# JeongsooP/RGB-no-more

Measured on AMD Instinct MI355X. Metric: images/sec JPEG-Ti DCT 512x512 train step, higher is better.
Workload: dtype bf16

## Files before the change

rgb-no-more_amd/csrc/vit_chain_bwd.hip:

```cpp
#include "common.h"
#include <string.h>
#include <type_traits>
#include "internal.h"
#include "ln_bwd_rows.h"
#include "chain_common.h"
#include "../../include/rgbnm.h"

namespace {

constexpr int E = 192, HID = 768, HD = 64, HEADS = 3, NTOK = 196, NTILE = 7, NPAD = 224, INNER = HEADS * HD, LDQ = 3 * INNER;
constexpr int NCW = 7, NTHREADS = 64 * (NCW + 1), CTHREADS = 64 * NCW, BM = 32 * NCW;
constexpr int ARR = NPAD * ROWB, SLOT = 24576, STAGE = 2 * SLOT, CH = 64, NCHUNK = HID / CH;
constexpr int CP = E + 4;
constexpr int SMEM = 163840;
constexpr int PIPE_P = 6, PIPE_M1 = 5, PIPE_X = 7;
constexpr int M_STG = 2 * STAGE;
constexpr int TILE = 32 * ROWB;
typedef rgbnm::LnBwdRows<CTHREADS, BM> LnBwd;
constexpr int RED_OFF = (BM * CP * 2 + 1023) / 1024 * 1024;
static_assert(RED_OFF + LnBwd::RED_BYTES <= 132096, "LDS");
constexpr int P_SLOT0 = 132096, P_SLOT1 = 0, P_TILES = 98304;
static_assert(P_SLOT0 + SLOT <= SMEM && P_TILES + NCW * TILE <= P_SLOT0, "LDS");
constexpr int A_Q = 0, A_K = ARR, A_V = 2 * ARR, A_G = 3 * ARR, A_L2 = 4 * ARR, A_D = A_L2 + NPAD * 4, A_STG = A_D + NPAD * 4;
constexpr int A_SIDE = A_STG + NCW * STG_WAVE;
static_assert(A_SIDE + NCW * 1024 <= SMEM, "LDS");
constexpr int X_SLOT0 = A_K, X_SLOT1 = A_K + SLOT, X_SLOT2 = 0, X_TILES = A_K + 2 * SLOT, X_TSET = NCW * TILE;
static_assert(X_SLOT1 + SLOT <= X_TILES && X_TILES + 3 * X_TSET <= SMEM && SLOT <= A_K, "LDS");

struct BwdBlk {
  const bf16* wimg;
  const float *ln1_g, *ln2_g;
  const bf16* x_in; const float *mean1, *rstd1;
  const bf16* qkv; const float* lse; const bf16* attn; const bf16* x_mid; const float *mean2, *rstd2; const bf16* gp;
  const bf16* dy;
  bf16* du; bf16* dx_mid; bf16* dqkv; bf16* dx;
  float *part2, *part1;
};
static_assert(sizeof(BwdBlk) == sizeof(rgbnm_chain_bwd_block), "rgbnm_chain_bwd_block layout");
constexpr int MAX_DEPTH = 12;
struct BwdArgs {
  BwdBlk blk[MAX_DEPTH]; bf16* dattn;
  int depth, nimg;
  float scale;
};

__device__ __forceinline__ void store_du(bf16* ptr, const bf16x8& v) { __builtin_nontemporal_store(v, reinterpret_cast<bf16x8*>(ptr)); }

__device__ __forceinline__ void dma_row_tiles(const bf16* __restrict__ src, int ld, unsigned char* dst, int lane) {
#pragma unroll 4
  for (int i = 0; i < 28; ++i) {
    const int row = 8 * i + (lane >> 3), pc = lane & 7;
    const int lc = pc ^ (row & 7);
    const int srow = row < NTOK ? row : NTOK - 1;
    __builtin_amdgcn_global_load_lds((glb_ptr)(src + (size_t)srow * ld + lc * 8), (lds_ptr)(dst + i * 1024), 16, 0, 0);
  }
}

__device__ __forceinline__ void tile_out(unsigned char* smem, unsigned stg, const u32x4& p0, const u32x4& p1, const u32x4& p2,
                                         const u32x4& p3, bf16* dst, int ld, int live) {
  const int ln = lane_id_here();
  const unsigned wo = stg + (unsigned)((ln & 31) * ROWB + (((ln >> 5) ^ (ln & 7)) << 4));
  *reinterpret_cast<u32x4*>(smem + wo) = p0;
  *reinterpret_cast<u32x4*>(smem + (wo ^ 32u)) = p1;
  *reinterpret_cast<u32x4*>(smem + (wo ^ 64u)) = p2;
  *reinterpret_cast<u32x4*>(smem + (wo ^ 96u)) = p3;
  own_tile_fence();
  const int rl = ln >> 3, seg = ln & 7;
  const unsigned ro = stg + (unsigned)(rl * ROWB + ((seg ^ rl) << 4));
  bf16* gp = dst + (size_t)rl * ld + seg * 8;
  u32x4 v[4];
#pragma unroll
  for (int i = 0; i < 4; ++i) v[i] = *reinterpret_cast<const u32x4*>(smem + ro + i * 8 * ROWB);
  if (live == 32) {
#pragma unroll
    for (int i = 0; i < 4; ++i) *reinterpret_cast<u32x4*>(gp + (size_t)i * 8 * ld) = v[i];
  } else {
#pragma unroll
    for (int i = 0; i < 4; ++i)
      if (i * 8 + rl < live) *reinterpret_cast<u32x4*>(gp + (size_t)i * 8 * ld) = v[i];
  }
  own_tile_fence();
}

__device__ __forceinline__ void tiles_write(const u32x4 (&v)[NTILE][4], bf16* __restrict__ g0, size_t ld, int lane) {
  const int rl = lane >> 3, seg = lane & 7;
#pragma unroll
  for (int wv = 0; wv < NTILE; ++wv)
#pragma unroll
    for (int i = 0; i < 4; ++i) {
      const int row = wv * 32 + i * 8 + rl;
      if (row < NTOK) *reinterpret_cast<u32x4*>(g0 + (size_t)row * ld + seg * 8) = v[wv][i];
    }
}

#ifdef CHAINB_PROF
__device__ unsigned long long g_chainb_prof[8 * 8 * 128];
#define CP_(i)                                                                                          \
  do {                                                                                                  \
    if (ib == CHAINB_PROF_BLK && blockIdx.x < 8) {                                                      \
      const unsigned long long t_ = __builtin_amdgcn_s_memtime();                                       \
      if ((threadIdx.x & 63) == 0) g_chainb_prof[(blockIdx.x * 8 + (threadIdx.x >> 6)) * 128 + (i)] = t_; \
    }                                                                                                   \
  } while (0)
#ifndef CHAINB_PROF_BLK
#define CHAINB_PROF_BLK 6
#endif
#else
#define CP_(i) do {} while (0)
#endif
#define BAR(s) do { CP_(2 * (s)); wg_barrier(); CP_(2 * (s) + 1); } while (0)
constexpr int B_M0 = 0;
constexpr int B_E2 = 12;
constexpr int B_P = 19;
constexpr int B_A = 24;
constexpr int B_X = 37;
constexpr int B_E1 = 46;
constexpr int B_END = 53;

__device__ __forceinline__ void ln_bwd_request(LnBwd& lnb, const bf16* X, const float* mean, const float* rstd, const bf16* R, int img,
                                               int w) {
  const int tid = w * 64 + lane_id_here();
  lnb.request_x(X, E, mean, rstd, img * NTOK, NTOK, tid);
  lnb.request_res(R, E, img * NTOK, NTOK, tid);
}
template <int B0>
__device__ __forceinline__ void ln_bwd_epilogue(unsigned char* smem, const f32x16 (&acc)[6], const bf16* X, const float* mean,
                                                const float* rstd, const bf16* R, const float* gamma, bf16* DX,
                                                float* part, int img, int w, int ib) {
  const int lane_ = lane_id_here();
  const int tid = w * 64 + lane_, rloc = w * 32 + (lane_ & 31), g = lane_ >> 5;
  LnBwd lnb;
  lnb.request_x(X, E, mean, rstd, img * NTOK, NTOK, tid);
  lnb.request_res(R, E, img * NTOK, NTOK, tid);
  wait_lds();
  BAR(B0);
  bf16* Cs = reinterpret_cast<bf16*>(smem);
#pragma unroll
  for (int b = 0; b < 6; ++b)
#pragma unroll
    for (int q = 0; q < 4; ++q) {
      const int nl = 32 * b + 8 * q + 4 * g;
      const f32x4 v = {acc[b][4 * q + 0], acc[b][4 * q + 1], acc[b][4 * q + 2], acc[b][4 * q + 3]};
      store4<bf16>(Cs + rloc * CP + nl, v);
    }
  wait_lds();
  BAR(B0 + 1);
  lnb.run<true>(Cs, CP, DX, E, gamma, true, part, img, reinterpret_cast<float*>(smem + RED_OFF), img * NTOK, NTOK, tid, Cs,
          [&](int k) { if (k == 0) BAR(B0 + 2); else if (k == 1) BAR(B0 + 3); else if (k == 2) BAR(B0 + 4); else BAR(B0 + 5); });
  wait_lds();
  BAR(B0 + 6);
}
__device__ __forceinline__ void read_own_rows(const unsigned char* smem, int w, Rows& x) {
  const int lane_ = lane_id_here();
  const unsigned char* rp = smem + (w * 32 + (lane_ & 31)) * (CP * 2) + 16 * (lane_ >> 5);
#pragma unroll
  for (int c = 0; c < 12; ++c) {
    const u32x2 lo = *reinterpret_cast<const u32x2*>(rp + 32 * c), hi = *reinterpret_cast<const u32x2*>(rp + 32 * c + 8);
    x.v[c] = u32x4{lo[0], lo[1], hi[0], hi[1]};
  }
}

__global__ __launch_bounds__(NTHREADS) void vit_chain_bwd_kernel(BwdArgs p) {
  extern __shared__ __attribute__((aligned(16))) unsigned char smem[];
  const int img = blockIdx.x;
  if (img >= p.nimg) return;
  const int w = __builtin_amdgcn_readfirstlane(threadIdx.x >> 6);
  const int depth = p.depth;

  if (w == NCW) {
    const int lane = threadIdx.x & 63;
    for (int ib = depth - 1; ib >= 0; --ib) {
      const BwdBlk& b = p.blk[ib];
      const unsigned char* wimg = reinterpret_cast<const unsigned char*>(b.wimg);
      dma_linear<48>(wimg, smem, lane);
      for (int c = 0; c < NCHUNK; ++c) {
        wait_vm<0>();
        BAR(B_M0 + c);
        if (c + 1 < NCHUNK) dma_linear<48>(wimg + (size_t)(c + 1) * STAGE, smem + ((c + 1) & 1) * STAGE, lane);
      }
      BAR(B_E2);
      dma_linear<24>(wimg + (size_t)NCHUNK * STAGE, smem + P_SLOT0, lane);
#pragma unroll
      for (int k = 1; k < 7; ++k) BAR(B_E2 + k);
      const bf16* qkv0 = b.qkv + (size_t)img * NTOK * LDQ;
      const bf16* do0 = p.dattn + (size_t)img * NTOK * INNER;
      bf16* dq0 = b.dqkv + (size_t)img * NTOK * LDQ;
      const unsigned char* stg0 = smem + A_STG;
      auto issue_kv = [&](int h) {
        dma_matrix_all(qkv0 + INNER + h * HD, LDQ, NTOK, smem + A_K, lane);
        dma_matrix_all(qkv0 + 2 * INNER + h * HD, LDQ, NTOK, smem + A_V, lane);
      };
      auto issue_q = [&](int h) { dma_matrix_all(qkv0 + h * HD, LDQ, NTOK, smem + A_Q, lane); };
      auto issue_g = [&](int h) { dma_matrix_all(do0 + h * HD, INNER, NTOK, smem + A_G, lane); };
      const unsigned char* xw = wimg + (size_t)NCHUNK * STAGE + 3 * SLOT;
      auto issue_xt = [&](int j) { dma_row_tiles(dq0 + j * 64, LDQ, smem + X_TILES + (j % 3) * X_TSET, lane); };
      wait_vm<0>();
      BAR(B_P);
      BAR(B_P + 1);
      dma_linear<24>(wimg + (size_t)NCHUNK * STAGE + SLOT, smem + P_SLOT1, lane);
      issue_kv(0);
      wait_vm<56>(); BAR(B_P + 2);
      dma_linear<24>(wimg + (size_t)NCHUNK * STAGE + 2 * SLOT, smem + P_SLOT0, lane);
      wait_vm<0>(); BAR(B_P + 3);
      issue_q(0);
      BAR(B_P + 4);
      {
        issue_g(0);
        wait_vm<0>();
        BAR(B_A);
        for (int h = 0; h < HEADS; ++h) {
          bf16* g0 = dq0 + h * HD;
          wait_vm<0>();
          BAR(B_A + 1 + 4 * h);
          u32x4 tq[NTILE][4];
          tiles_read<true>(stg0, NTOK, lane, tq);
          wait_lds();
          BAR(B_A + 2 + 4 * h);
          tiles_write(tq, g0, LDQ, lane);
          if (h + 1 < HEADS) issue_kv(h + 1);
          else {
            dma_linear<24>(xw, smem + X_SLOT0, lane);
            dma_linear<24>(xw + SLOT, smem + X_SLOT1, lane);
          }
          wait_vm<0>();
          BAR(B_A + 3 + 4 * h);
          tiles_read<true>(stg0, NTOK, lane, tq);
          wait_lds();
          BAR(B_A + 4 + 4 * h);
          tiles_write(tq, g0 + INNER, LDQ, lane);
          tiles_read<false>(smem + A_G, NTOK, lane, tq);
          wait_lds();
          if (h + 1 < HEADS) {
            issue_q(h + 1);
            issue_g(h + 1);
          } else {
            issue_xt(0);
          }
          tiles_write(tq, g0 + 2 * INNER, LDQ, lane);
        }
      }
      for (int j = 0; j < 9; ++j) {
        if (j == 0) wait_vm<28>();
        else if (j + 1 < 9) wait_vm<52>();
        else wait_vm<0>();
        BAR(B_X + j);
        if (j == 0) {
          issue_xt(1);
          dma_linear<24>(xw + 2 * SLOT, smem + X_SLOT2, lane);
          issue_xt(2);
        }
        if (j + 2 < 9 && j >= 1) {
          dma_linear<24>(xw + (size_t)(j + 2) * SLOT, smem + ((j + 2) % 3 == 0 ? X_SLOT0 : ((j + 2) % 3 == 1 ? X_SLOT1 : X_SLOT2)), lane);
          issue_xt(j + 2);
        }
      }
#pragma unroll
      for (int k = 0; k < 7; ++k) BAR(B_E1 + k);
      BAR(B_END);
    }
    return;
  }

  const int row0 = 32 * w;
  const int live = NTOK - row0 < 32 ? NTOK - row0 : 32;
  const size_t grow0 = (size_t)img * NTOK + row0;
  const float LOG2E = 1.4426950408889634f;
  const float c2 = p.scale * LOG2E;

  Rows dyf;
  {
    const int lane_ = lane_id_here();
    const int rloc = row0 + (lane_ & 31), tok = rloc < NTOK ? rloc : NTOK - 1;
    const bf16* yrow = p.blk[depth - 1].dy + ((size_t)img * NTOK + tok) * E + 8 * (lane_ >> 5);
#pragma unroll
    for (int c = 0; c < 12; ++c) dyf.v[c] = *reinterpret_cast<const u32x4*>(yrow + 16 * c);
  }

  for (int ib = depth - 1; ib >= 0; --ib) {
    const BwdBlk& b = p.blk[ib];
    f32x16 acc2[6];
#pragma unroll
    for (int bt = 0; bt < 6; ++bt)
#pragma unroll
      for (int r = 0; r < 16; ++r) acc2[bt][r] = 0.f;
    {
      const Geo L = fresh_geo();
      const int fl = L.fl;
      const int woff0 = L.l31 * (E * 2) + ((L.g ^ fl) << 4);
      const unsigned stg = (unsigned)(M_STG + w * 2 * TILE);
      bf16x8 gpraw[4];
      auto load_gp = [&](int chunk) {
        const int ln = lane_id_here();
#pragma unroll
        for (int i = 0; i < 4; ++i) {
          const int idx = ln + 64 * i, row = idx >> 3, vec = idx & 7;
          int rr = row0 + row;
          rr = rr < NTOK ? rr : NTOK - 1;
          const bf16x8* gsrc = reinterpret_cast<const bf16x8*>(b.gp + ((size_t)img * NTOK + rr) * HID + chunk * CH + vec * 8);
          gpraw[i] = *gsrc;
        }
      };
      load_gp(0);
      for (int chunk = 0; chunk < NCHUNK; ++chunk) {
        {
          const int ln = lane_id_here();
#pragma unroll
          for (int i = 0; i < 4; ++i) {
            const int idx = ln + 64 * i, row = idx >> 3, vec = idx & 7;
            *reinterpret_cast<bf16x8*>(smem + stg + row * ROWB + ((vec ^ (row & 7)) << 4)) = gpraw[i];
          }
        }
        if (chunk + 1 < NCHUNK) load_gp(chunk + 1);
        wait_lds();
        BAR(B_M0 + chunk);
        const unsigned st_off = (unsigned)((chunk & 1) * STAGE);
        const unsigned char* sW1 = smem + st_off;
        const unsigned w2o = opaque(st_off + (unsigned)(SLOT + L.l31 * ROWB + ((L.g ^ fl) << 4)));
        const unsigned two = opaque(stg + (unsigned)(L.l31 * ROWB + ((L.g ^ (L.l31 & 7)) << 4)));
#pragma unroll
        for (int ht = 0; ht < 2; ++ht) {
          f32x16 a1;
#pragma unroll
          for (int r = 0; r < 16; ++r) a1[r] = 0.f;
          int wbase = woff0 + ht * 32 * (E * 2);
          asm volatile("" : "+v"(wbase));
          {
            Frag<bf16> fb[12];
#pragma unroll
            for (int c = 0; c < 12; ++c)
              fb[c].v = *reinterpret_cast<const bf16x8*>(sW1 + ((wbase ^ ((c % 4) << 5)) + 128 * (c / 4)));
#pragma unroll
            for (int c = 0; c < 12; ++c) {
              Frag<bf16> fx;
              fx.v = as_bf16x8(dyf.v[c]);
              mma(a1, fb[c], fx);
            }
            __builtin_amdgcn_sched_group_barrier(0x100, PIPE_M1, 0);
#pragma unroll
            for (int i = 0; i < 12 - PIPE_M1; ++i) {
              __builtin_amdgcn_sched_group_barrier(0x008, 1, 0);
              __builtin_amdgcn_sched_group_barrier(0x100, 1, 0);
            }
#pragma unroll
            for (int i = 0; i < PIPE_M1; ++i) __builtin_amdgcn_sched_group_barrier(0x008, 1, 0);
            __builtin_amdgcn_sched_barrier(0);
          }
          Frag<bf16> fw2[12];
#pragma unroll
          for (int bt = 0; bt < 6; ++bt)
            fw2[bt].v = *reinterpret_cast<const bf16x8*>(smem + (w2o ^ (unsigned)((2 * ht) << 5)) + bt * 32 * ROWB);
          __builtin_amdgcn_sched_barrier(0);
          Frag<bf16> pg[2];
#pragma unroll
          for (int hs = 0; hs < 2; ++hs) {
            const unsigned to = two ^ (unsigned)((2 * ht + hs) << 5);
            const bf16x8 gpv = *reinterpret_cast<const bf16x8*>(smem + to);
            bf16x8 dv;
#pragma unroll
            for (int j = 0; j < 8; ++j) dv[j] = (bf16)((float)(bf16)a1[8 * hs + j] * (float)gpv[j]);
            pg[hs].v = dv;
            *reinterpret_cast<bf16x8*>(smem + to + TILE) = dv;
          }
          __builtin_amdgcn_sched_barrier(0);
#pragma unroll
          for (int bt = 0; bt < 6; ++bt)
            fw2[6 + bt].v = *reinterpret_cast<const bf16x8*>(smem + (w2o ^ (unsigned)((2 * ht + 1) << 5)) + bt * 32 * ROWB);
#pragma unroll
          for (int bt = 0; bt < 6; ++bt) mma(acc2[bt], fw2[bt], pg[0]);
#pragma unroll
          for (int bt = 0; bt < 6; ++bt) mma(acc2[bt], fw2[6 + bt], pg[1]);
#pragma unroll
          for (int i = 0; i < 6; ++i) {
            __builtin_amdgcn_sched_group_barrier(0x008, 1, 0);
            __builtin_amdgcn_sched_group_barrier(0x100, 1, 0);
          }
          __builtin_amdgcn_sched_group_barrier(0x008, 6, 0);
          __builtin_amdgcn_sched_barrier(0);
        }
        own_tile_fence();
        const int ln = lane_id_here();
        bf16x8 dv0[4];
#pragma unroll
        for (int i = 0; i < 4; ++i) {
          const int idx = ln + 64 * i, row = idx >> 3, vec = idx & 7;
          dv0[i] = *reinterpret_cast<const bf16x8*>(smem + stg + TILE + row * ROWB + ((vec ^ (row & 7)) << 4));
        }
        if (live == 32) {
#pragma unroll
          for (int i = 0; i < 4; ++i) {
            const int idx = ln + 64 * i, row = idx >> 3, vec = idx & 7;
            store_du(b.du + (grow0 + row) * HID + chunk * CH + vec * 8, dv0[i]);
          }
        } else {
#pragma unroll
          for (int i = 0; i < 4; ++i) {
            const int idx = ln + 64 * i, row = idx >> 3, vec = idx & 7;
            if (row < live) store_du(b.du + (grow0 + row) * HID + chunk * CH + vec * 8, dv0[i]);
          }
        }
      }
    }
    ln_bwd_epilogue<B_E2>(smem, acc2, b.x_mid, b.mean2, b.rstd2, b.dy, b.ln2_g, b.dx_mid, b.part2, img, w, ib);
    {
      const Geo L = fresh_geo();
      Rows dxf;
      read_own_rows(smem, w, dxf);
      wait_lds();
      BAR(B_P);
      const unsigned stg = (unsigned)(P_TILES + w * TILE);
#pragma unroll
      for (int h = 0; h < HEADS; ++h) {
        BAR(B_P + 1 + h);
        const unsigned char* sW = smem + (h == 1 ? P_SLOT1 : P_SLOT0);
        f32x16 acc[2];
#pragma unroll
        for (int ht = 0; ht < 2; ++ht)
#pragma unroll
          for (int r = 0; r < 16; ++r) acc[ht][r] = 0.f;
        gemm_k192x2<PIPE_P, true>(acc[0], acc[1], sW, dxf, L);
        u32x4 pc[4];
#pragma unroll
        for (int ht = 0; ht < 2; ++ht)
#pragma unroll
          for (int hs = 0; hs < 2; ++hs)
#pragma unroll
            for (int d = 0; d < 4; ++d) pc[2 * ht + hs][d] = pack2(acc[ht][8 * hs + 2 * d], acc[ht][8 * hs + 2 * d + 1]);
        tile_out(smem, stg, pc[0], pc[1], pc[2], pc[3], p.dattn + grow0 * INNER + h * HD, INNER, live);
      }
      asm volatile("s_waitcnt vmcnt(0)" ::: "memory");
      BAR(B_P + 4);
    }
    {
      unsigned char* Qs = smem + A_Q;
      unsigned char* Ks = smem + A_K;
      unsigned char* Vs = smem + A_V;
      unsigned char* Gs = smem + A_G;
      float* L2_s = reinterpret_cast<float*>(smem + A_L2);
      float* D_s = reinterpret_cast<float*>(smem + A_D);
      unsigned char* stg = smem + A_STG + w * STG_WAVE;
      const Geo L = fresh_geo();
      const int fl = L.fl;
      const unsigned rb0 = (unsigned)(L.l31 * ROWB + ((L.g ^ fl) << 4));
      const int row = row0 + L.l31;
      u32x4 qraw[4], graw[4], oraw[4];
      float lq = 0.f;
      const bf16* qkv0 = b.qkv + (size_t)img * NTOK * LDQ;
      const bf16* do0 = p.dattn + (size_t)img * NTOK * INNER;
      const bf16* o0 = b.attn + (size_t)img * NTOK * INNER;
      auto load_own_g = [&](int h) {
        const int lane_ = lane_id_here();
        const int seg = lane_ & 7;
#pragma unroll
        for (int i = 0; i < 4; ++i) {
          int r = row0 + i * 8 + (lane_ >> 3);
          r = r < NTOK ? r : NTOK - 1;
          graw[i] = *reinterpret_cast<const u32x4*>(do0 + (size_t)r * INNER + h * HD + seg * 8);
        }
      };
      unsigned char* qside = smem + A_SIDE + w * 1024;
      auto load_own_q = [&](int h) {
        const int lane_ = lane_id_here();
        const int seg = lane_ & 7;
#pragma unroll
        for (int i = 0; i < 4; ++i) {
          int r = row0 + i * 8 + (lane_ >> 3);
          r = r < NTOK ? r : NTOK - 1;
          const bf16* src = qkv0 + (size_t)r * LDQ + h * HD + seg * 8;
          if (i == 0) __builtin_amdgcn_global_load_lds((glb_ptr)src, (lds_ptr)qside, 16, 0, 0);
          else qraw[i] = *reinterpret_cast<const u32x4*>(src);
        }
      };
      auto load_own_o = [&](int h) {
        const int lane_ = lane_id_here();
        const int seg = lane_ & 7;
#pragma unroll
        for (int i = 0; i < 4; ++i) {
          int r = row0 + i * 8 + (lane_ >> 3);
          r = r < NTOK ? r : NTOK - 1;
          oraw[i] = *reinterpret_cast<const u32x4*>(o0 + (size_t)r * INNER + h * HD + seg * 8);
        }
        int rq_ = row0 + (lane_ & 31);
        rq_ = rq_ < NTOK ? rq_ : NTOK - 1;
        lq = b.lse[((size_t)img * HEADS + h) * NTOK + rq_];
      };
      load_own_g(0);
      load_own_q(0);
      load_own_o(0);
      BAR(B_A);
      for (int h = 0; h < HEADS; ++h) {
        const bool more = h + 1 < HEADS;
        asm volatile("s_waitcnt vmcnt(0)" ::: "memory");
        Frag<bf16> kf[4], vf[4];
        {
          f32x16 dq[2];
          Frag<bf16> qf[4], gf[4];
          const int rl = L.lane >> 3, seg = L.lane & 7;
#pragma unroll
          for (int i = 0; i < 4; ++i) {
            const bf16x8 gv = __builtin_bit_cast(bf16x8, graw[i]), ov = __builtin_bit_cast(bf16x8, oraw[i]);
            float d = 0.f;
#pragma unroll
            for (int e = 0; e < 8; ++e) d += (float)gv[e] * (float)ov[e];
            d += lane_xor1(d);
            d += lane_xor2(d);
            d += lane_xor4(d);
            if (seg == 0) D_s[row0 + i * 8 + rl] = d;
          }
          qraw[0] = *reinterpret_cast<const u32x4*>(qside + lane_id_here() * 16);
#pragma unroll
          for (int i = 0; i < 4; ++i) *reinterpret_cast<u32x4*>(stg + (i * 8 + rl) * STG_PITCH + seg * 16) = qraw[i];
          own_tile_fence();
#pragma unroll
          for (int c = 0; c < 4; ++c) qf[c].v = *reinterpret_cast<const bf16x8*>(stg + L.l31 * STG_PITCH + (2 * c + L.g) * 16);
          own_tile_fence();
#pragma unroll
          for (int i = 0; i < 4; ++i) *reinterpret_cast<u32x4*>(stg + (i * 8 + rl) * STG_PITCH + seg * 16) = graw[i];
          own_tile_fence();
#pragma unroll
          for (int c = 0; c < 4; ++c) gf[c].v = *reinterpret_cast<const bf16x8*>(stg + L.l31 * STG_PITCH + (2 * c + L.g) * 16);
          const float Dq = D_s[row];
          own_tile_fence();
          const float lq2 = lq * LOG2E;
          if (L.g == 0) L2_s[row] = lq2;
#pragma unroll
          for (int dt = 0; dt < 2; ++dt)
#pragma unroll
            for (int r = 0; r < 16; ++r) dq[dt][r] = 0.f;
          unsigned rb = rb0, tr = L.tr0;
          asm volatile("" : "+v"(rb), "+v"(tr));
          const unsigned kt = (unsigned)A_K + tr;
          TileLoop<NTILE>::run([&](auto tc) {
            constexpr int t = decltype(tc)::value;
            f32x16 sa, da;
#pragma unroll
            for (int r = 0; r < 16; ++r) { sa[r] = 0.f; da[r] = 0.f; }
            row_pair_mma(sa, da, Ks, Vs, rb, t, qf, gf);
            float ds[16];
#pragma unroll
            for (int r = 0; r < 16; ++r) {
              const float pr = __builtin_amdgcn_exp2f(fmaf(sa[r], c2, -lq2));
              ds[r] = pr * (da[r] - Dq);
            }
            if (t * 32 + 32 > NTOK) {
#pragma unroll
              for (int r = 0; r < 16; ++r)
                if (t * 32 + acc_row(r, L.lane) >= NTOK) ds[r] = 0.f;
            }
            Frag<bf16> kk[4];
            tfrag4<t>(kt, kk);
            Frag<bf16> sf = pfrag<bf16>(ds, 0);
            mma(dq[0], kk[0], sf);
            mma(dq[1], kk[1], sf);
            sf = pfrag<bf16>(ds, 1);
            mma(dq[0], kk[2], sf);
            mma(dq[1], kk[3], sf);
          });
          tile_park_private(stg, dq, p.scale, L);
#pragma unroll
          for (int c = 0; c < 4; ++c) {
            kf[c] = rowfrag_x(Ks, rb, w, c);
            vf[c] = rowfrag_x(Vs, rb, w, c);
          }
        }
        wait_lds();
        BAR(B_A + 1 + 4 * h);
        BAR(B_A + 2 + 4 * h);
        {
          f32x16 dk[2], dv[2];
#pragma unroll
          for (int dt = 0; dt < 2; ++dt)
#pragma unroll
            for (int r = 0; r < 16; ++r) { dk[dt][r] = 0.f; dv[dt][r] = 0.f; }
          unsigned rb = rb0, tr = L.tr0;
          asm volatile("" : "+v"(rb), "+v"(tr));
          const unsigned qt_ = (unsigned)A_Q + tr, gt_ = (unsigned)A_G + tr;
          TileLoop<NTILE>::run([&](auto tc) {
            constexpr int t = decltype(tc)::value;
            f32x16 sa, da;
#pragma unroll
            for (int r = 0; r < 16; ++r) { sa[r] = 0.f; da[r] = 0.f; }
            row_pair_mma(sa, da, Qs, Gs, rb, t, kf, vf);
            float pp[16], ds[16];
#pragma unroll
            for (int q4 = 0; q4 < 4; ++q4) {
              const f32x4 l4 = *reinterpret_cast<const f32x4*>(L2_s + t * 32 + 8 * q4 + 4 * L.g);
              const f32x4 d4 = *reinterpret_cast<const f32x4*>(D_s + t * 32 + 8 * q4 + 4 * L.g);
#pragma unroll
              for (int e = 0; e < 4; ++e) {
                const int r = 4 * q4 + e;
                const float pr = __builtin_amdgcn_exp2f(fmaf(sa[r], c2, -l4[e]));
                pp[r] = pr;
                ds[r] = pr * (da[r] - d4[e]);
              }
            }
            if (t * 32 + 32 > NTOK) {
#pragma unroll
              for (int r = 0; r < 16; ++r)
                if (t * 32 + acc_row(r, L.lane) >= NTOK) { pp[r] = 0.f; ds[r] = 0.f; }
            }
            Frag<bf16> gg[4];
            tfrag4<t>(gt_, gg);
            Frag<bf16> f = pfrag<bf16>(pp, 0);
            mma(dv[0], gg[0], f);
            mma(dv[1], gg[1], f);
            f = pfrag<bf16>(pp, 1);
            mma(dv[0], gg[2], f);
            mma(dv[1], gg[3], f);
            tfrag4<t>(qt_, gg);
            f = pfrag<bf16>(ds, 0);
            mma(dk[0], gg[0], f);
            mma(dk[1], gg[1], f);
            f = pfrag<bf16>(ds, 1);
            mma(dk[0], gg[2], f);
            mma(dk[1], gg[3], f);
          });
          if (more) load_own_g(h + 1);
          tile_park_private(stg, dk, p.scale, L);
          if (more) load_own_q(h + 1);
          wait_lds();
          BAR(B_A + 3 + 4 * h);
          tile_park_rows(Gs, w, dv, 1.0f);
        }
        if (more) load_own_o(h + 1);
        wait_lds();
        BAR(B_A + 4 + 4 * h);
      }
    }
    f32x16 accx[6];
#pragma unroll
    for (int bt = 0; bt < 6; ++bt)
#pragma unroll
      for (int r = 0; r < 16; ++r) accx[bt][r] = 0.f;
    for (int j = 0; j < 9; ++j) {
      BAR(B_X + j);
      const Geo L = fresh_geo();
      const int fl = L.fl;
      const int set = j % 3;
      const unsigned wo = opaque((unsigned)((set == 0 ? X_SLOT0 : (set == 1 ? X_SLOT1 : X_SLOT2)) + L.l31 * ROWB + ((L.g ^ fl) << 4)));
      const unsigned to = opaque((unsigned)(X_TILES + set * X_TSET + w * TILE + L.l31 * ROWB + ((L.g ^ (L.l31 & 7)) << 4)));
#pragma unroll
      for (int s = 0; s < 4; ++s) {
        Frag<bf16> fx, fw[6];
        fx.v = *reinterpret_cast<const bf16x8*>(smem + (to ^ (unsigned)(s << 5)));
#pragma unroll
        for (int bt = 0; bt < 6; ++bt)
          fw[bt].v = *reinterpret_cast<const bf16x8*>(smem + (wo ^ (unsigned)(s << 5)) + bt * 32 * ROWB);
#pragma unroll
        for (int bt = 0; bt < 6; ++bt) mma(accx[bt], fw[bt], fx);
      }
      __builtin_amdgcn_sched_group_barrier(0x100, PIPE_X, 0);
#pragma unroll
      for (int i = 0; i < 24; ++i) {
        __builtin_amdgcn_sched_group_barrier(0x008, 1, 0);
        if (i < 28 - PIPE_X) __builtin_amdgcn_sched_group_barrier(0x100, 1, 0);
      }
      __builtin_amdgcn_sched_barrier(0);
    }
    ln_bwd_epilogue<B_E1>(smem, accx, b.x_in, b.mean1, b.rstd1, b.dx_mid, b.ln1_g, b.dx, b.part1, img, w, ib);
    read_own_rows(smem, w, dyf);
    wait_lds();
    BAR(B_END);
  }
}

}

#ifdef CHAINB_PROF
extern "C" int rgbnm_chainb_prof_read(unsigned long long* host_out) {
  return hipMemcpyFromSymbol(host_out, HIP_SYMBOL(g_chainb_prof), sizeof(unsigned long long) * 8 * 8 * 128) == hipSuccess ? 0 : -1;
}
#endif

extern "C" {

size_t rgbnm_chain_bwd_block_bytes(void) { return sizeof(BwdBlk); }

int rgbnm_vit_chain_bwd(const rgbnm_vit_cfg* c, const rgbnm_chain_bwd_block* blocks, int depth, void* dattn, void* stream) {
  if (!c || !blocks || !dattn || depth <= 0) return RGBNM_EINVAL;
  if (c->dtype != RGBNM_DT_BF16 || c->E != E || c->heads != HEADS || c->N != NTOK || c->B < 1 || depth > MAX_DEPTH) return 1;
  BwdArgs p;
  memcpy(p.blk, blocks, sizeof(BwdBlk) * depth);
  p.dattn = (bf16*)dattn; p.depth = depth; p.nimg = c->B; p.scale = c->attn_scale;
  static DevOnce attr;
  if (attr.need()) {
    if (hipFuncSetAttribute((const void*)vit_chain_bwd_kernel, hipFuncAttributeMaxDynamicSharedMemorySize, SMEM) != hipSuccess)
      return RGBNM_ELAUNCH;
    attr.done();
  }
  const double tok = (double)c->B * NTOK;
  const double flops = depth * tok * 2.0 * (2.0 * E * HID + INNER * E + 3.0 * INNER * E + 4.0 * NTOK * INNER);
  const double bytes = depth * (tok * ((2.0 * HID + 5.0 * E + 2.0 * 3.0 * INNER) * 2.0 + 4 * 4 + HEADS * 4) + 36.0 * SLOT) + tok * E * 2.0;
  const int slot = rgbnm_trace_begin(TR_CHAIN_BWD, flops, bytes, (hipStream_t)stream);
  hipLaunchKernelGGL(vit_chain_bwd_kernel, dim3(c->B), dim3(NTHREADS), SMEM, (hipStream_t)stream, p);
  rgbnm_trace_end(slot, (hipStream_t)stream);
  LAUNCH_CHECK();
  return RGBNM_OK;
}

}
```

Baseline: 68000.

## Reorder projection heads so last-head dattn stays in LDS and registers

The backward projection now processes heads in a rotated order (1,2,0), so head 0's dattn tile is produced last. That tile is written straight into the attention G buffer in LDS and kept in registers (graw). This replaces the later global reload of dattn for head 0 and the DMA issue_g(0). It also drops a vmcnt(0) wait in favour of an LDS wait, and clamps row reads. Risks include correctness on padded rows, changed swizzle assumptions, and higher register pressure.

```diff
diff --git a/rgb-no-more_amd/csrc/vit_chain_bwd.hip b/rgb-no-more_amd/csrc/vit_chain_bwd.hip
--- a/rgb-no-more_amd/csrc/vit_chain_bwd.hip
+++ b/rgb-no-more_amd/csrc/vit_chain_bwd.hip
@@ -27,6 +27,8 @@
 constexpr int X_SLOT0 = A_K, X_SLOT1 = A_K + SLOT, X_SLOT2 = 0, X_TILES = A_K + 2 * SLOT, X_TSET = NCW * TILE;
 static_assert(X_SLOT1 + SLOT <= X_TILES && X_TILES + 3 * X_TSET <= SMEM && SLOT <= A_K, "LDS");
 
+constexpr int p_head(int s) { return (s + 1) % HEADS; }
+
 struct BwdBlk {
   const bf16* wimg;
   const float *ln1_g, *ln2_g;
@@ -71,6 +73,31 @@
   u32x4 v[4];
 #pragma unroll
   for (int i = 0; i < 4; ++i) v[i] = *reinterpret_cast<const u32x4*>(smem + ro + i * 8 * ROWB);
+  if (live == 32) {
+#pragma unroll
+    for (int i = 0; i < 4; ++i) *reinterpret_cast<u32x4*>(gp + (size_t)i * 8 * ld) = v[i];
+  } else {
+#pragma unroll
+    for (int i = 0; i < 4; ++i)
+      if (i * 8 + rl < live) *reinterpret_cast<u32x4*>(gp + (size_t)i * 8 * ld) = v[i];
+  }
+  own_tile_fence();
+}
+
+__device__ __forceinline__ void tile_keep_out(unsigned char* smem, unsigned rows, const u32x4& p0, const u32x4& p1, const u32x4& p2,
+                                              const u32x4& p3, u32x4 (&v)[4], bf16* dst, int ld, int live) {
+  const int ln = lane_id_here();
+  const unsigned wo = rows + (unsigned)((ln & 31) * ROWB + (((ln >> 5) ^ fswz(ln & 31)) << 4));
+  *reinterpret_cast<u32x4*>(smem + wo) = p0;
+  *reinterpret_cast<u32x4*>(smem + (wo ^ 32u)) = p1;
+  *reinterpret_cast<u32x4*>(smem + (wo ^ 64u)) = p2;
+  *reinterpret_cast<u32x4*>(smem + (wo ^ 96u)) = p3;
+  own_tile_fence();
+  const int rl = ln >> 3, seg = ln & 7;
+  bf16* gp = dst + (size_t)rl * ld + seg * 8;
+#pragma unroll
+  for (int i = 0; i < 4; ++i)
+    v[i] = *reinterpret_cast<const u32x4*>(smem + rows + (unsigned)((i * 8 + rl) * ROWB + ((seg ^ fswz(i * 8 + rl)) << 4)));
   if (live == 32) {
 #pragma unroll
     for (int i = 0; i < 4; ++i) *reinterpret_cast<u32x4*>(gp + (size_t)i * 8 * ld) = v[i];
@@ -150,9 +177,12 @@
   wait_lds();
   BAR(B0 + 6);
 }
+template <bool CLAMP = false>
 __device__ __forceinline__ void read_own_rows(const unsigned char* smem, int w, Rows& x) {
   const int lane_ = lane_id_here();
-  const unsigned char* rp = smem + (w * 32 + (lane_ & 31)) * (CP * 2) + 16 * (lane_ >> 5);
+  int r = w * 32 + (lane_ & 31);
+  if (CLAMP) r = r < NTOK ? r : NTOK - 1;
+  const unsigned char* rp = smem + r * (CP * 2) + 16 * (lane_ >> 5);
 #pragma unroll
   for (int c = 0; c < 12; ++c) {
     const u32x2 lo = *reinterpret_cast<const u32x2*>(rp + 32 * c), hi = *reinterpret_cast<const u32x2*>(rp + 32 * c + 8);
@@ -179,7 +209,7 @@
         if (c + 1 < NCHUNK) dma_linear<48>(wimg + (size_t)(c + 1) * STAGE, smem + ((c + 1) & 1) * STAGE, lane);
       }
       BAR(B_E2);
-      dma_linear<24>(wimg + (size_t)NCHUNK * STAGE, smem + P_SLOT0, lane);
+      dma_linear<24>(wimg + (size_t)NCHUNK * STAGE + p_head(0) * SLOT, smem + P_SLOT0, lane);
 #pragma unroll
       for (int k = 1; k < 7; ++k) BAR(B_E2 + k);
       const bf16* qkv0 = b.qkv + (size_t)img * NTOK * LDQ;
@@ -197,15 +227,14 @@
       wait_vm<0>();
       BAR(B_P);
       BAR(B_P + 1);
-      dma_linear<24>(wimg + (size_t)NCHUNK * STAGE + SLOT, smem + P_SLOT1, lane);
+      dma_linear<24>(wimg + (size_t)NCHUNK * STAGE + p_head(1) * SLOT, smem + P_SLOT1, lane);
       issue_kv(0);
       wait_vm<56>(); BAR(B_P + 2);
-      dma_linear<24>(wimg + (size_t)NCHUNK * STAGE + 2 * SLOT, smem + P_SLOT0, lane);
+      dma_linear<24>(wimg + (size_t)NCHUNK * STAGE + p_head(2) * SLOT, smem + P_SLOT0, lane);
       wait_vm<0>(); BAR(B_P + 3);
       issue_q(0);
       BAR(B_P + 4);
       {
-        issue_g(0);
         wait_vm<0>();
         BAR(B_A);
         for (int h = 0; h < HEADS; ++h) {
@@ -401,17 +430,19 @@
       }
     }
     ln_bwd_epilogue<B_E2>(smem, acc2, b.x_mid, b.mean2, b.rstd2, b.dy, b.ln2_g, b.dx_mid, b.part2, img, w, ib);
+    u32x4 graw[4];
     {
       const Geo L = fresh_geo();
       Rows dxf;
-      read_own_rows(smem, w, dxf);
+      read_own_rows<true>(smem, w, dxf);
       wait_lds();
       BAR(B_P);
       const unsigned stg = (unsigned)(P_TILES + w * TILE);
 #pragma unroll
-      for (int h = 0; h < HEADS; ++h) {
-        BAR(B_P + 1 + h);
-        const unsigned char* sW = smem + (h == 1 ? P_SLOT1 : P_SLOT0);
+      for (int s = 0; s < HEADS; ++s) {
+        const int h = p_head(s);
+        BAR(B_P + 1 + s);
+        const unsigned char* sW = smem + (s == 1 ? P_SLOT1 : P_SLOT0);
         f32x16 acc[2];
 #pragma unroll
         for (int ht = 0; ht < 2; ++ht)
@@ -425,9 +456,11 @@
           for (int hs = 0; hs < 2; ++hs)
 #pragma unroll
             for (int d = 0; d < 4; ++d) pc[2 * ht + hs][d] = pack2(acc[ht][8 * hs + 2 * d], acc[ht][8 * hs + 2 * d + 1]);
-        tile_out(smem, stg, pc[0], pc[1], pc[2], pc[3], p.dattn + grow0 * INNER + h * HD, INNER, live);
+        if (s == HEADS - 1)
+          tile_keep_out(smem, (unsigned)(A_G + w * TILE), pc[0], pc[1], pc[2], pc[3], graw, p.dattn + grow0 * INNER + h * HD, INNER, live);
+        else tile_out(smem, stg, pc[0], pc[1], pc[2], pc[3], p.dattn + grow0 * INNER + h * HD, INNER, live);
       }
-      asm volatile("s_waitcnt vmcnt(0)" ::: "memory");
+      wait_lds();
       BAR(B_P + 4);
     }
     {
@@ -442,7 +475,7 @@
       const int fl = L.fl;
       const unsigned rb0 = (unsigned)(L.l31 * ROWB + ((L.g ^ fl) << 4));
       const int row = row0 + L.l31;
-      u32x4 qraw[4], graw[4], oraw[4];
+      u32x4 qraw[4], oraw[4];
       float lq = 0.f;
       const bf16* qkv0 = b.qkv + (size_t)img * NTOK * LDQ;
       const bf16* do0 = p.dattn + (size_t)img * NTOK * INNER;
@@ -483,7 +516,6 @@
         rq_ = rq_ < NTOK ? rq_ : NTOK - 1;
         lq = b.lse[((size_t)img * HEADS + h) * NTOK + rq_];
       };
-      load_own_g(0);
       load_own_q(0);
       load_own_o(0);
       BAR(B_A);
```

Result: no change. 68110 (median of 3 runs) (+0.2%).
